# urgent-challenge/urgent2026_challenge_track1

Hardware: AMD Instinct MI355X
Metric: utterances/sec (4 s @ 48 kHz) train step (higher is better)
Workload: dtype bf16

## Files before the change

urgent2026_challenge_track1_amd/csrc/gemm.hip:

```cpp
#include <stdlib.h>

#include <type_traits>
#include "urse_common.h"

namespace urse {

typedef __bf16 bf16x8_t __attribute__((ext_vector_type(8)));
typedef short short8_t __attribute__((ext_vector_type(8)));
typedef short short4_t __attribute__((ext_vector_type(4)));
typedef float f32x4_t __attribute__((ext_vector_type(4)));

struct GemmDesc {
  const char* A;
  const char* B;
  char* C;
  const float* bias;
  const float* resid;
  long lda, ldb, ldc;
  long M, N, K;
  long ldr;
};

constexpr int BM = 128, BN = 128;
constexpr int SLAB = 64;
// ... 1409 lines not shown
        const long row = m0 + pass * RPP + lr_;
        const bool ok = slot < SLOTS && col < d.N && lr_ < RPP && row < d.M;
        gnb_xpre[i] = ok ? *reinterpret_cast<const float4*>(xt->gnb_x + row * d.ldc + col) : make_float4(0.f, 0.f, 0.f, 0.f);
      }
      if (slot < SLOTS && col < d.N) {
#pragma unroll
        for (int i = 0; i < XI; ++i) {
          const int lr_ = slot + i * SLOTS;
          const long row = m0 + pass * RPP + lr_;
          if (lr_ < RPP && row < d.M) {
            const float4 f = *reinterpret_cast<const float4*>(lds + lr_ * CP + chf * 16);
            __builtin_nontemporal_store(*reinterpret_cast<const f32x4_t*>(&f), reinterpret_cast<f32x4_t*>(C + row * d.ldc + col));
            const float4 xv = gnb_xpre[i];
            const bool first = row < gnb_bound;
            const float mean = first ? gnb_m[0] : gnb_m[1], rstd = first ? gnb_r[0] : gnb_r[1];
            const float dy[4] = {f.x, f.y, f.z, f.w}, xs[4] = {xv.x, xv.y, xv.z, xv.w};
            float a1 = 0.f, a2 = 0.f;
#pragma unroll
            for (int q = 0; q < 4; ++q) {
              const float xh = (xs[q] - mean) * rstd;
              gnb_dg[q] += dy[q] * xh;
              gnb_db[q] += dy[q];
              a1 += dy[q] * gnb_ga[q];
              a2 += dy[q] * gnb_ga[q] * xh;
            }
            if (first) { gsa += a1; gqa += a2; } else { gsb += a1; gqb += a2; }
          }
        }
      }
      continue;
    }
    int lrow = tid / CPR, ch = tid - lrow * CPR;
    constexpr int DROW = NTHR / CPR, DCH = NTHR - DROW * CPR;
    for (; lrow < RPP; lrow += DROW) {
      const long row = m0 + pass * RPP + lrow, col = n0 + ch * EPC;
      if (row < d.M && col < d.N) {
        const char* src = lds + lrow * CP + ch * 16;
        if (vec_ok && col + EPC <= d.N) {
          uint4 v = *reinterpret_cast<const uint4*>(src);
          if (OS == 4 && d.resid && ACT != 2) {
            const float4 rr = *reinterpret_cast<const float4*>(d.resid + row * d.ldr + col);
            float4 f = *reinterpret_cast<float4*>(&v);
            f.x += rr.x; f.y += rr.y; f.z += rr.z; f.w += rr.w;
            v = *reinterpret_cast<uint4*>(&f);
          }
          if (gst) {
            const float4 f = *reinterpret_cast<const float4*>(&v);
            const float sv = (f.x + f.y) + (f.z + f.w), qv = (f.x * f.x + f.y * f.y) + (f.z * f.z + f.w * f.w);
            if (row < gbound) { gsa += sv; gqa += qv; } else { gsb += sv; gqb += qv; }
          }
#ifdef NABL_NO_GST
          if (v.x == 0x12345678u)
#endif
          __builtin_nontemporal_store(*reinterpret_cast<const f32x4_t*>(&v), reinterpret_cast<f32x4_t*>(C + row * d.ldc + col));
          if constexpr (C2K) {
            if (C2) {
              float a0, a1, a2, a3, a4, a5, a6, a7;
              unpack2<f16_t>(v.x, a0, a1); unpack2<f16_t>(v.y, a2, a3); unpack2<f16_t>(v.z, a4, a5); unpack2<f16_t>(v.w, a6, a7);
              const uint4 o = make_uint4(pack2<bf16_t>(a0, a1), pack2<bf16_t>(a2, a3), pack2<bf16_t>(a4, a5), pack2<bf16_t>(a6, a7));
              __builtin_nontemporal_store(*reinterpret_cast<const f32x4_t*>(&o), reinterpret_cast<f32x4_t*>(C2 + row * d.ldr + col));
            }
          }
        } else {
          const TO* sv = reinterpret_cast<const TO*>(src);
          for (int e = 0; e < EPC && col + e < d.N; ++e) {
            float f = to_f32<TO>(sv[e]);
            if (OS == 4 && d.resid && ACT != 2) f += d.resid[row * d.ldr + col + e];
            if (gst) {
              if (row < gbound) { gsa += f; gqa += f * f; } else { gsb += f; gqb += f * f; }
            }
            C[row * d.ldc + col + e] = from_f32<TO>(f);
            if constexpr (C2K) {
              if (C2) C2[row * d.ldr + col + e] = f32_to_bf16(f);
            }
          }
        }
      }
      ch += DCH;
      if (ch >= CPR) { ch -= CPR; ++lrow; }
    }
  }
  if constexpr (GNB) {
    __syncthreads();
    constexpr int SLOTS = NTHR / CPR;
    double* red = reinterpret_cast<double*>(lds);
    float4* pg = reinterpret_cast<float4*>(lds + 1024);
    float4* pb = pg + SLOTS * CPR;
    const double r0 = wave_sum_d((double)gsa), r1 = wave_sum_d((double)gqa), r2 = wave_sum_d((double)gsb), r3 = wave_sum_d((double)gqb);
    if (lane == 0) { red[w * 4] = r0; red[w * 4 + 1] = r1; red[w * 4 + 2] = r2; red[w * 4 + 3] = r3; }
    if (tid < SLOTS * CPR) {
      pg[tid] = make_float4(gnb_dg[0], gnb_dg[1], gnb_dg[2], gnb_dg[3]);
      pb[tid] = make_float4(gnb_db[0], gnb_db[1], gnb_db[2], gnb_db[3]);
    }
    __syncthreads();
    if (tid < 4) {
      double t = 0.0;
      for (int i = 0; i < NWV; ++i) t += red[i * 4 + tid];
      const long g = gnb_g0 + (tid >> 1);
      if ((tid < 2 || gnb_bound < m0 + BMX) && g * xt->rpg < d.M) atomicAdd(xt->gnb_sums + g * 2 + (tid & 1), t);
    }
    if (tid >= 64 && tid < 64 + CPR) {
      const int chf = tid - 64;
      const long col = n0 + chf * EPC;
      if (col < d.N) {
        float4 sg = make_float4(0.f, 0.f, 0.f, 0.f), sb = sg;
        for (int i = 0; i < SLOTS; ++i) {
          const float4 a = pg[i * CPR + chf], bq = pb[i * CPR + chf];
          sg.x += a.x; sg.y += a.y; sg.z += a.z; sg.w += a.w;
          sb.x += bq.x; sb.y += bq.y; sb.z += bq.z; sb.w += bq.w;
        }
        float* part = xt->gnb_part + (long)(blockIdx.x % xt->gnb_slots) * 2 * d.N;
        const float vg[4] = {sg.x, sg.y, sg.z, sg.w}, vb[4] = {sb.x, sb.y, sb.z, sb.w};
        for (int q = 0; q < 4 && col + q < d.N; ++q) {
          atomicAdd(part + col + q, vg[q]);
          atomicAdd(part + d.N + col + q, vb[q]);
        }
      }
    }
    return;
  }
  if (gst) {
    __syncthreads();
    double* red = reinterpret_cast<double*>(lds);
    const double r0 = wave_sum_d((double)gsa), r1 = wave_sum_d((double)gqa), r2 = wave_sum_d((double)gsb), r3 = wave_sum_d((double)gqb);
    if (lane == 0) { red[w * 4] = r0; red[w * 4 + 1] = r1; red[w * 4 + 2] = r2; red[w * 4 + 3] = r3; }
    __syncthreads();
    if (tid < 4) {
      double t = 0.0;
      for (int i = 0; i < NWV; ++i) t += red[i * 4 + tid];
      const long g = gidx + (tid >> 1);
      if (tid < 2 || gbound < m0 + BMX) {
        if (g * rpg < d.M) atomicAdd(gstats + g * 2 + (tid & 1), t);
      }
    }
  }
}

template <typename TO, int NTW, int ACT, int BMX, int WNC = 2, typename TI = bf16_t>
__global__ void __launch_bounds__(BMX / 64 * WNC * 64) gemm_nt_dma_kernel(GemmDesc d, NtExtra x) {
  gemm_nt_dma_body<TO, NTW, ACT, BMX, WNC, 0, TI>(d, x.gstats, x.rpg);
}

__global__ void __launch_bounds__(512) gemm_nt_dma_gnb_kernel(GemmDesc d, NtExtra x) {
  gemm_nt_dma_body<float, 7, 0, 256, 2, 1>(d, nullptr, 0, &x);
}

__global__ void gnb_fold_kernel(const float* __restrict__ part, int slots, int N, float* __restrict__ dgamma, float* __restrict__ dbeta) {
  const int c = blockIdx.x * blockDim.x + threadIdx.x;
  if (c >= N) return;
  float a = 0.f, b = 0.f;
  for (int s = 0; s < slots; ++s) { a += part[(long)s * 2 * N + c]; b += part[(long)s * 2 * N + N + c]; }
  dgamma[c] += a;
  dbeta[c] += b;
}

template <typename TO, int ACT, typename TI = bf16_t>
__global__ void __launch_bounds__(512) gemm_nt_dma_grouped_kernel(const GemmDesc* __restrict__ descs) {
  const GemmDesc d = descs[blockIdx.y];
  gemm_nt_dma_body<TO, 7, ACT, 256, 2, 0, TI>(d);
}

template <int ACT, typename TI = bf16_t>
__global__ void __launch_bounds__(512) gemm_nt_bres_kernel(GemmDesc d, int wg_per_slice) {
  constexpr int BMX = 256, NTW = 7, BNX = 224, NST = 3, STAGE = BMX * 64, KSTEPS = 7, BRES = KSTEPS * 14 * 1024;
  __shared__ __attribute__((aligned(1024))) char lds[BRES + NST * STAGE];
  char* ring = lds + BRES;
  const int tm = (int)((d.M + BMX - 1) / BMX);
  const int tile_n = blockIdx.x / wg_per_slice, part = blockIdx.x - tile_n * wg_per_slice;
  const long n0 = (long)tile_n * BNX;
  const int tid = threadIdx.x, lane = tid & 63;
  const int w = __builtin_amdgcn_readfirstlane(tid >> 6), wm = w >> 1, wn = w & 1;
  const int nk = (int)(d.K / 32);
  const char* zsrc = reinterpret_cast<const char*>(g_tn_zero_page) + lane * 16;
  const int srow = lane >> 2, schunk = (lane & 3) ^ ((lane >> 3) & 3);
  const int lc = lane & 15, lr = lane >> 4;
  const int foff = lc * 64 + ((lr ^ ((lc >> 1) & 3)) << 4);
  for (int blk = w; blk < nk * 14; blk += 8) {
    const int kt = blk / 14, b = blk - kt * 14;
    const long row = n0 + b * 16 + srow;
    glds16(row < d.N ? d.B + (row * d.ldb) * 2 + schunk * 16 + (long)kt * 64 : zsrc, lds + blk * 1024);
  }
  f32x4_t bv[NTW];
#pragma unroll
  for (int j = 0; j < NTW; ++j) {
    const long col = n0 + (wn * NTW + j) * 16 + lr * 4;
#pragma unroll
    for (int r = 0; r < 4; ++r) bv[j][r] = (d.bias && col + r < d.N) ? d.bias[col + r] : 0.f;
  }
  bf16_t* C = reinterpret_cast<bf16_t*>(d.C);
  auto tile_src = [&](int mt, const char* (&pa)[2], bool (&aok)[2]) __attribute__((always_inline)) {
#pragma unroll
    for (int j = 0; j < 2; ++j) {
      const long row = (long)mt * BMX + 16 * (2 * w + j) + srow;
      aok[j] = mt < tm && row < d.M;
      pa[j] = d.A + (row * d.lda) * 2 + schunk * 16;
    }
  };
  auto issue = [&](const char* (&pa)[2], bool (&aok)[2], int kt, int slot) __attribute__((always_inline)) {
#pragma unroll
    for (int j = 0; j < 2; ++j)
      glds16((kt < nk && aok[j]) ? pa[j] + (long)kt * 64 : zsrc, ring + slot * STAGE + (2 * w + j) * 1024);
  };
  const char* pa[2];
  bool aok[2];
  tile_src(part, pa, aok);
  issue(pa, aok, 0, 2);
  for (int mt = part; mt < tm; mt += wg_per_slice) {
    const long m0 = (long)mt * BMX;
    issue(pa, aok, 1, 0);
    f32x4_t acc[4][NTW];
#pragma unroll
    for (int i = 0; i < 4; ++i)
#pragma unroll
      for (int j = 0; j < NTW; ++j) acc[i][j] = f32x4_t{0.f, 0.f, 0.f, 0.f};
    int slot = 2;
    for (int kt = 0; kt < nk; ++kt) {
      asm volatile("s_waitcnt vmcnt(2)" ::: "memory");
      __builtin_amdgcn_s_barrier();
      int nslot = slot + 2;
      if (nslot >= NST) nslot -= NST;
      issue(pa, aok, kt + 2, nslot);
      const char* As = ring + slot * STAGE + wm * 4096 + foff;
      const char* Bs = lds + kt * (14 * 1024) + wn * NTW * 1024 + foff;
      short8_t a[4], b[NTW];
#pragma unroll
      for (int i = 0; i < 4; ++i) a[i] = *reinterpret_cast<const short8_t*>(As + i * 1024);
#pragma unroll
      for (int j = 0; j < NTW; ++j) b[j] = *reinterpret_cast<const short8_t*>(Bs + j * 1024);
#pragma unroll
      for (int j = 0; j < NTW; ++j)
#pragma unroll
        for (int i = 0; i < 4; ++i) acc[i][j] = Frag<TI>::mma(b[j], a[i], acc[i][j]);
      if (++slot == NST) slot = 0;
    }
    asm volatile("s_waitcnt vmcnt(0)" ::: "memory");
    __syncthreads();
    tile_src(mt + wg_per_slice, pa, aok);
    issue(pa, aok, 0, 2);
    constexpr int CP = BNX * 2 + 16, RPP = 64, CPR = BNX / 8, DROW = 512 / CPR, DCH = 512 - DROW * CPR;
    static_assert(RPP * CP <= 2 * STAGE, "staging must leave slot 2 alone");
#pragma unroll 1
    for (int pass = 0; pass < BMX / RPP; ++pass) {
      if (pass > 0) {
        asm volatile("s_waitcnt lgkmcnt(0)" ::: "memory");
        __builtin_amdgcn_s_barrier();
      }
      if (wm == pass) {
#pragma unroll
        for (int j = 0; j < NTW; ++j) {
          const int lcol = (wn * NTW + j) * 16 + lr * 4;
#pragma unroll
          for (int i = 0; i < 4; ++i) {
            f32x4_t v = acc[i][j] + bv[j];
            if (ACT == 1) {
#pragma unroll
              for (int r = 0; r < 4; ++r) v[r] = tanhf_(v[r]);
            }
            uint2 pk;
            pk.x = pack2<TI>(v[0], v[1]);
            pk.y = pack2<TI>(v[2], v[3]);
            *reinterpret_cast<uint2*>(ring + (i * 16 + lc) * CP + lcol * 2) = pk;
          }
        }
      }
      asm volatile("s_waitcnt lgkmcnt(0)" ::: "memory");
      __builtin_amdgcn_s_barrier();
      int lrow = tid / CPR, ch = tid - lrow * CPR;
      for (; lrow < RPP; lrow += DROW) {
        const long row = m0 + pass * RPP + lrow, col = n0 + ch * 8;
        if (row < d.M && col < d.N) {
          const char* src = ring + lrow * CP + ch * 16;
          if (col + 8 <= d.N) {
            __builtin_nontemporal_store(*reinterpret_cast<const f32x4_t*>(src), reinterpret_cast<f32x4_t*>(C + row * d.ldc + col));
          } else {
            const bf16_t* sv = reinterpret_cast<const bf16_t*>(src);
            for (int e = 0; e < 8 && col + e < d.N; ++e) C[row * d.ldc + col + e] = sv[e];
          }
        }
        ch += DCH;
        if (ch >= CPR) { ch -= CPR; ++lrow; }
      }
    }
    asm volatile("s_waitcnt lgkmcnt(0)" ::: "memory");
    __builtin_amdgcn_s_barrier();
  }
  asm volatile("s_waitcnt vmcnt(0)" ::: "memory");
}

#ifdef URSE_EXPERIMENTS
constexpr int WR_ROWS = 32, WR_KS = 7, WR_NSLOT = 7, WR_STAGE = WR_KS * 2 * 1024, WR_BNX = 448, WR_CP = WR_BNX * 2 + 16, WR_AHEAD = WR_NSLOT - 1;
template <int ACT>
__global__ void __launch_bounds__(448) gemm_nt_wreg_kernel(GemmDesc d, int parts, long rows_per_part) {
  __shared__ __attribute__((aligned(1024))) char lds[WR_NSLOT * WR_STAGE + 2 * WR_ROWS * WR_CP];
  char* outs = lds + WR_NSLOT * WR_STAGE;
  const int tn_ = (int)gridDim.x / parts;
  const int lid = xcd_remap((int)blockIdx.x, (int)gridDim.x);
  const int part = lid / tn_, tile_n = lid - part * tn_;
  const long n0 = (long)tile_n * WR_BNX;
  const long r_begin = (long)part * rows_per_part;
  long r_end = r_begin + rows_per_part;
  if (r_end > d.M) r_end = d.M;
  if (r_begin >= r_end) return;
  const int nst = (int)((r_end - r_begin + WR_ROWS - 1) / WR_ROWS);
  const int tid = threadIdx.x, lane = tid & 63;
  const int w = __builtin_amdgcn_readfirstlane(tid >> 6);
  const int lc = lane & 15, lr = lane >> 4;
// ... 86 lines not shown
#endif
    }
    char* ob = outs + (k & 1) * (WR_ROWS * WR_CP);
#pragma unroll
    for (int i = 0; i < 2; ++i)
#pragma unroll
      for (int j = 0; j < 4; ++j) {
        f32x4_t v = acc[i][j] + bv[j];
        if (ACT == 1) {
#pragma unroll
          for (int r = 0; r < 4; ++r) v[r] = tanhf_(v[r]);
        }
        uint2 pk;
        pk.x = (unsigned)f32_to_bf16(v[0]) | ((unsigned)f32_to_bf16(v[1]) << 16);
        pk.y = (unsigned)f32_to_bf16(v[2]) | ((unsigned)f32_to_bf16(v[3]) << 16);
        *reinterpret_cast<uint2*>(ob + (i * 16 + lc) * WR_CP + (w * 64 + j * 16 + lr * 4) * 2) = pk;
      }
    {
      const int kk = k < 6 ? k : 6;
      switch (kk) {
        case 0: asm volatile("s_waitcnt vmcnt(10)" ::: "memory"); break;
        case 1: asm volatile("s_waitcnt vmcnt(14)" ::: "memory"); break;
        case 2: asm volatile("s_waitcnt vmcnt(18)" ::: "memory"); break;
        case 3: asm volatile("s_waitcnt vmcnt(22)" ::: "memory"); break;
        case 4: asm volatile("s_waitcnt vmcnt(26)" ::: "memory"); break;
        case 5: asm volatile("s_waitcnt vmcnt(30)" ::: "memory"); break;
        default: asm volatile("s_waitcnt vmcnt(34)" ::: "memory"); break;
      }
    }
    static_assert(WR_AHEAD == 6 && NPC == 4, "the counted waits above are written for six stages ahead and four stores per sweep");
    asm volatile("s_waitcnt lgkmcnt(0)" ::: "memory");
    __builtin_amdgcn_s_barrier();
  }
  sweep(nst - 1);
}
#endif

static int check_desc_host(const GemmDesc& d, int es, const char* who) {
  URSE_CHECK_ARG(d.A && d.B && d.C, "%s: null operand", who);
  URSE_CHECK_ARG(d.M > 0 && d.N > 0 && d.K > 0, "%s: empty problem", who);
  URSE_CHECK_ARG((d.K * es) % SLAB == 0, "%s: K (%ld) must be a multiple of %d elements", who, d.K, SLAB / es);
  URSE_CHECK_ARG((d.lda * es) % 16 == 0 && (d.ldb * es) % 16 == 0 && ((uintptr_t)d.A % 16) == 0 &&
                     ((uintptr_t)d.B % 16) == 0,
                 "%s: operands must be 16-byte aligned with 16-byte-multiple row pitch", who);
  URSE_CHECK_ARG(d.lda >= d.K && d.ldb >= d.K && d.ldc >= d.N, "%s: leading dimension too small", who);
  return URSE_OK;
}

template <typename T, typename TO>
static void launch_nt(const GemmDesc* descs, const GemmDesc& single, int groups, int max_blocks, int act,
                      hipStream_t st) {
  hipLaunchKernelGGL((gemm_nt_kernel<T, TO>), dim3(max_blocks, 1, groups), dim3(256), 0, st, descs, single, act);
}

static int dispatch_nt(const GemmDesc* descs, const GemmDesc& single, int groups, int max_blocks, int in_dtype,
                       int out_dtype, int act, hipStream_t st) {
  if (in_dtype == URSE_BF16 && out_dtype == URSE_BF16) launch_nt<bf16_t, bf16_t>(descs, single, groups, max_blocks, act, st);
  else if (in_dtype == URSE_BF16 && out_dtype == URSE_F32) launch_nt<bf16_t, float>(descs, single, groups, max_blocks, act, st);
  else if (in_dtype == URSE_F32 && out_dtype == URSE_F32) launch_nt<float, float>(descs, single, groups, max_blocks, act, st);
  else if (in_dtype == URSE_F32 && out_dtype == URSE_BF16) launch_nt<float, bf16_t>(descs, single, groups, max_blocks, act, st);
  else if (in_dtype == URSE_F16 && out_dtype == URSE_F16) launch_nt<f16_t, f16_t>(descs, single, groups, max_blocks, act, st);
  else if (in_dtype == URSE_F16 && out_dtype == URSE_F32) launch_nt<f16_t, float>(descs, single, groups, max_blocks, act, st);
  else { set_error("gemm_nt: bad dtype %d/%d", in_dtype, out_dtype); return URSE_ERR_INVALID_ARG; }
  URSE_CHECK_LAUNCH("urse_gemm_nt");
  return URSE_OK;
}

static long g_nt_bres_min_n = getenv("URSE_NT_BRES_MIN_N") ? atol(getenv("URSE_NT_BRES_MIN_N")) : 448;
static int g_nt_bres_wgs = 256;
static int g_nt_wide_default = 1;
static long g_nt_wide_maxk = 256;

static int gemm_nt_impl(const void* A, int64_t lda, const void* B, int64_t ldb, void* C, int64_t ldc,
                        const float* bias, const float* resid, int64_t ldr, int64_t M, int64_t N, int64_t K,
                        int in_dtype, int out_dtype, int act, void* stream, double* gstats, long rpg, int* fused) {
  NtExtra xtra{};
  GemmDesc d;
  d.A = (const char*)A; d.B = (const char*)B; d.C = (char*)C; d.bias = bias; d.resid = resid;
  d.lda = lda; d.ldb = ldb; d.ldc = ldc; d.M = M; d.N = N; d.K = K; d.ldr = ldr;
  const bool in16 = in_dtype == URSE_BF16 || in_dtype == URSE_F16;
  const bool f16 = in_dtype == URSE_F16;
  URSE_CHECK_ARG(in16 || in_dtype == URSE_F32, "urse_gemm_nt: bad operand dtype %d", in_dtype);
  URSE_CHECK_ARG(out_dtype == URSE_F32 || (out_dtype == URSE_BF16 && !f16) || (out_dtype == URSE_F16 && f16),
                 "urse_gemm_nt: output dtype %d with operand dtype %d (16-bit outputs take the operands' format)", out_dtype, in_dtype);
  const bool out16 = out_dtype != URSE_F32;
  int rc = check_desc_host(d, in16 ? 2 : 4, "urse_gemm_nt");
  if (rc) return rc;
  URSE_CHECK_ARG(!resid || act == 2 || out_dtype == URSE_F32 || (in_dtype == URSE_F16 && out_dtype == URSE_F16 && act == 1),
                 "urse_gemm_nt: residual epilogue writes f32 (f16 operands with act 1: the aux slot is the bf16 copy of the output)");
  URSE_CHECK_ARG(act != 2 || resid, "urse_gemm_nt: act 2 (tanh backward) needs the aux operand");
  static const bool no_dma = getenv("URSE_NT_NO_DMA") != nullptr;
  const char* bres_env = getenv("URSE_NT_BRES");
  const int bres_mode = bres_env ? atoi(bres_env) : 1;
#ifdef URSE_EXPERIMENTS
  const long wreg_min_n = getenv("URSE_NT_WREG_MIN_N") ? atol(getenv("URSE_NT_WREG_MIN_N")) : 0;
  if (wreg_min_n > 0 && in_dtype == URSE_BF16 && out_dtype == URSE_BF16 && !no_dma && M >= 8192 && N >= wreg_min_n && K == 32 * WR_KS &&
      !resid && act != 2 && (ldc * 2) % 16 == 0 && ((uintptr_t)C % 16) == 0 && M * lda * 2 < 0xFFFFF000L && M * ldc * 2 < 0xFFFFF000L) {
    const int tn = (int)((N + WR_BNX - 1) / WR_BNX);
    int parts = 252 / tn;
    if (parts < 1) parts = 1;
    long rpp = (M + parts - 1) / parts;
    rpp = (rpp + WR_ROWS - 1) / WR_ROWS * WR_ROWS;
    dim3 grid((unsigned)(tn * parts));
    hipStream_t st = (hipStream_t)stream;
    note_launch(URSE_KV_NT_BRES);
    if (act == 0) hipLaunchKernelGGL(gemm_nt_wreg_kernel<0>, grid, dim3(448), 0, st, d, parts, rpp);
    else hipLaunchKernelGGL(gemm_nt_wreg_kernel<1>, grid, dim3(448), 0, st, d, parts, rpp);
    URSE_CHECK_LAUNCH("urse_gemm_nt");
    return URSE_OK;
  }
#endif
  if (bres_mode && in16 && out16 && !no_dma && M >= 8192 && N >= g_nt_bres_min_n && K % 32 == 0 &&
      K >= 96 && K <= 224 && !resid && act != 2 && (ldc * 2) % 16 == 0 && ((uintptr_t)C % 16) == 0) {
    const int tn = (int)((N + 223) / 224);
    int per = g_nt_bres_wgs / tn;
    if (per < 1) per = 1;
    dim3 grid((unsigned)(tn * per));
    hipStream_t st = (hipStream_t)stream;
    note_launch(URSE_KV_NT_BRES);
    if (f16) {
      if (act == 0) hipLaunchKernelGGL((gemm_nt_bres_kernel<0, f16_t>), grid, dim3(512), 0, st, d, per);
      else hipLaunchKernelGGL((gemm_nt_bres_kernel<1, f16_t>), grid, dim3(512), 0, st, d, per);
    } else if (act == 0) hipLaunchKernelGGL(gemm_nt_bres_kernel<0>, grid, dim3(512), 0, st, d, per);
    else hipLaunchKernelGGL(gemm_nt_bres_kernel<1>, grid, dim3(512), 0, st, d, per);
    URSE_CHECK_LAUNCH("urse_gemm_nt");
    return URSE_OK;
  }
  if (in16 && !no_dma && M >= 2048 && N >= 160 && K % 32 == 0 && K >= 96 && !(f16 && act == 2)) {
    const long pad7 = (N + 223) / 224 * 224, pad8 = (N + 255) / 256 * 256;
    int ntw = pad7 <= pad8 ? 7 : 8;
    if (const char* e = getenv("URSE_NT_NTW")) ntw = atoi(e) == 8 ? 8 : 7;
    int bmx = 256;
    if (const char* e = getenv("URSE_NT_BMX")) bmx = atoi(e) == 128 ? 128 : 256;
    int wide = g_nt_wide_default && K <= g_nt_wide_maxk && N >= 1792 && out_dtype == URSE_BF16 && (N + 447) / 448 * 448 <= pad7 + 64;
    if (const char* e = getenv("URSE_NT_WIDE")) wide = atoi(e) != 0 && N >= 448;
    if (f16) { wide = 0; bmx = 256; }
    const long tl = wide ? ((M + 127) / 128) * ((N + 447) / 448) : ((M + bmx - 1) / bmx) * ((N + 32L * ntw - 1) / (32L * ntw));
    URSE_CHECK_ARG(tl < (1L << 31), "urse_gemm_nt: too many tiles");
    dim3 grid((unsigned)tl);
    hipStream_t st = (hipStream_t)stream;
    if (gstats && out_dtype == URSE_F32 && act != 2 && !wide && rpg >= bmx) {
      xtra.gstats = gstats;
      xtra.rpg = rpg;
      if (fused) *fused = 1;
    }
#define URSE_NT_DMA(TO_, NTW_, ACT_, BMX_) \
  hipLaunchKernelGGL((gemm_nt_dma_kernel<TO_, NTW_, ACT_, BMX_>), grid, dim3(BMX_ * 2), 0, st, d, xtra)
#define URSE_NT_DMA_W(TO_, ACT_) \
  hipLaunchKernelGGL((gemm_nt_dma_kernel<TO_, 7, ACT_, 128, 4>), grid, dim3(512), 0, st, d, xtra)
#define URSE_NT_DMA_B(TO_, NTW_, ACT_) do { if (wide) URSE_NT_DMA_W(TO_, ACT_); else if (bmx == 128) URSE_NT_DMA(TO_, NTW_, ACT_, 128); else URSE_NT_DMA(TO_, NTW_, ACT_, 256); } while (0)
#define URSE_NT_DMA_ACT(TO_, NTW_) \
  do { if (act == 0) URSE_NT_DMA_B(TO_, NTW_, 0); else if (act == 1) URSE_NT_DMA_B(TO_, NTW_, 1); else URSE_NT_DMA_B(TO_, NTW_, 2); } while (0)
    note_launch(wide ? URSE_KV_NT_RING_WIDE : URSE_KV_NT_RING);
    if (f16) {
#define URSE_NT_DMA_H(TO_, NTW_, ACT_) hipLaunchKernelGGL((gemm_nt_dma_kernel<TO_, NTW_, ACT_, 256, 2, f16_t>), grid, dim3(512), 0, st, d, xtra)
#define URSE_NT_DMA_H_ACT(TO_, NTW_) do { if (act == 0) URSE_NT_DMA_H(TO_, NTW_, 0); else URSE_NT_DMA_H(TO_, NTW_, 1); } while (0)
      if (out_dtype == URSE_F16) { if (ntw == 7) URSE_NT_DMA_H_ACT(f16_t, 7); else URSE_NT_DMA_H_ACT(f16_t, 8); }
      else { if (ntw == 7) URSE_NT_DMA_H_ACT(float, 7); else URSE_NT_DMA_H_ACT(float, 8); }
    } else if (out_dtype == URSE_BF16) {
      if (ntw == 7) URSE_NT_DMA_ACT(bf16_t, 7); else URSE_NT_DMA_ACT(bf16_t, 8);
    } else {
      if (ntw == 7) URSE_NT_DMA_ACT(float, 7); else URSE_NT_DMA_ACT(float, 8);
    }
    URSE_CHECK_LAUNCH("urse_gemm_nt");
    return URSE_OK;
  }
  const long blocks = ((M + BM - 1) / BM) * ((N + BN - 1) / BN);
  URSE_CHECK_ARG(blocks < (1L << 31), "urse_gemm_nt: too many tiles");
  note_launch(URSE_KV_NT_128);
  return dispatch_nt(nullptr, d, 1, (int)blocks, in_dtype, out_dtype, act, (hipStream_t)stream);
}

extern "C" int urse_gemm_nt(const void* A, int64_t lda, const void* B, int64_t ldb, void* C, int64_t ldc,
                            const float* bias, const float* resid, int64_t ldr, int64_t M, int64_t N, int64_t K,
                            int in_dtype, int out_dtype, int act, void* stream) {
  return gemm_nt_impl(A, lda, B, ldb, C, ldc, bias, resid, ldr, M, N, K, in_dtype, out_dtype, act, stream, nullptr, 0, nullptr);
}

extern "C" int urse_gemm_nt_gnstats(const void* A, int64_t lda, const void* B, int64_t ldb, float* C, int64_t ldc,
                                    const float* bias, const float* resid, int64_t ldr, int64_t M, int64_t N, int64_t K,
                                    int in_dtype, int act, double* stats, int64_t rows_per_group, void* stream) {
  URSE_CHECK_ARG(stats && rows_per_group > 0 && M % rows_per_group == 0 && ldc == N && N % 4 == 0,
                 "urse_gemm_nt_gnstats: needs whole groups of rows, a dense output and N %% 4 == 0");
  const int groups = (int)(M / rows_per_group);
  (void)hipMemsetAsync(stats, 0, sizeof(double) * 2 * groups, (hipStream_t)stream);
  int fused = 0;
  int rc = gemm_nt_impl(A, lda, B, ldb, C, ldc, bias, resid, ldr, M, N, K, in_dtype, URSE_F32, act, stream, stats, rows_per_group,
                        &fused);
  if (rc || fused) return rc;
  return urse_groupnorm_stats(C, stats, groups, (int)rows_per_group, 1, (int)N, (int)N, stream);
}

extern "C" int urse_gemm_nt_gnbwd(const void* A, int64_t lda, const void* B, int64_t ldb, float* C, int64_t M, int64_t N, int64_t K,
                                  int in_dtype, const float* x, const double* stats, const float* gamma, double* sums, float* dgamma,
                                  float* dbeta, float* part, int slots, int64_t rows_per_group, float eps, void* stream) {
  URSE_CHECK_ARG(A && B && C && x && stats && gamma && sums && dgamma && dbeta && part && slots > 0 && rows_per_group > 0,
                 "urse_gemm_nt_gnbwd: bad argument");
  static const bool no_dma = getenv("URSE_NT_NO_DMA") != nullptr;
  if (no_dma || in_dtype != URSE_BF16 || M < 2048 || N < 160 || N > 224 || N % 4 || K % 32 || K < 96 || rows_per_group < 256 ||
      M % rows_per_group || ((uintptr_t)C % 16) || ((uintptr_t)x % 16)) {
    set_error("urse_gemm_nt_gnbwd: shape M%ld N%ld K%ld not served by the fused kernel", (long)M, (long)N, (long)K);
    return URSE_ERR_UNSUPPORTED;
  }
  GemmDesc d;
  d.A = (const char*)A; d.B = (const char*)B; d.C = (char*)C; d.bias = nullptr; d.resid = nullptr;
  d.lda = lda; d.ldb = ldb; d.ldc = N; d.M = M; d.N = N; d.K = K; d.ldr = 0;
  int rc = check_desc_host(d, 2, "urse_gemm_nt_gnbwd");
  if (rc) return rc;
  hipStream_t st = (hipStream_t)stream;
  const size_t sums_bytes = sizeof(double) * 2 * (size_t)(M / rows_per_group), part_bytes = sizeof(float) * 2 * (size_t)N * slots;
  if (reinterpret_cast<char*>(part) == reinterpret_cast<char*>(sums) + sums_bytes) {
    (void)hipMemsetAsync(sums, 0, sums_bytes + part_bytes, st);
  } else {
    (void)hipMemsetAsync(sums, 0, sums_bytes, st);
    (void)hipMemsetAsync(part, 0, part_bytes, st);
  }
  NtExtra xt{};
  xt.rpg = rows_per_group; xt.gnb_x = x; xt.gnb_stats = stats; xt.gnb_gamma = gamma; xt.gnb_sums = sums; xt.gnb_part = part;
  xt.gnb_slots = slots; xt.gnb_eps = eps;
  const long tl = (M + 255) / 256;
  URSE_CHECK_ARG(tl < (1L << 31), "urse_gemm_nt_gnbwd: too many tiles");
  note_launch(URSE_KV_NT_RING);
  hipLaunchKernelGGL(gemm_nt_dma_gnb_kernel, dim3((unsigned)tl), dim3(512), 0, st, d, xt);
  hipLaunchKernelGGL(gnb_fold_kernel, dim3((unsigned)((N + 255) / 256)), dim3(256), 0, st, part, slots, (int)N, dgamma, dbeta);
  URSE_CHECK_LAUNCH("urse_gemm_nt_gnbwd");
  return URSE_OK;
}

extern "C" int urse_gemm_nt_grouped(const void* descs, int groups, int max_blocks, int in_dtype, int out_dtype,
                                    int act, void* stream) {
  URSE_CHECK_ARG(descs && groups > 0 && max_blocks > 0, "urse_gemm_nt_grouped: bad argument");
  GemmDesc dummy;
  memset(&dummy, 0, sizeof(dummy));
  note_launch(URSE_KV_NT_GROUPED_128);
  return dispatch_nt((const GemmDesc*)descs, dummy, groups, max_blocks, in_dtype, out_dtype, act,
                     (hipStream_t)stream);
}

extern "C" int urse_gemm_nt_grouped_h(const void* descs, const int64_t* host_descs, int groups, int in_dtype,
                                      int out_dtype, int act, void* stream) {
  URSE_CHECK_ARG(descs && host_descs && groups > 0 && groups < 65536, "urse_gemm_nt_grouped_h: bad argument");
  const GemmDesc* hd = reinterpret_cast<const GemmDesc*>(host_descs);
  const bool f16 = in_dtype == URSE_F16;
  const int es = (in_dtype == URSE_BF16 || f16) ? 2 : 4;
  URSE_CHECK_ARG(out_dtype == URSE_F32 || (out_dtype == URSE_BF16 && !f16) || (out_dtype == URSE_F16 && f16),
                 "urse_gemm_nt_grouped_h: output dtype %d with operand dtype %d", out_dtype, in_dtype);
  bool dma = es == 2 && !(f16 && act == 2) && !getenv("URSE_NT_NO_DMA") && !getenv("URSE_NT_GROUPED_NO_DMA");
  long t128 = 0, tdma = 0;
  const char* mm = getenv("URSE_NT_GROUPED_MIN_M");
  const long min_m = mm ? atol(mm) : 1024;
  for (int g = 0; g < groups; ++g) {
    const GemmDesc& d = hd[g];
    if (int rc = check_desc_host(d, es, "urse_gemm_nt_grouped_h")) return rc;
    dma = dma && d.K % 32 == 0 && d.N >= 160 && d.M >= min_m;
    t128 = std::max(t128, ((d.M + BM - 1) / BM) * ((d.N + BN - 1) / BN));
    tdma = std::max(tdma, ((d.M + 255) / 256) * ((d.N + 223) / 224));
  }
  URSE_CHECK_ARG(t128 < (1L << 31), "urse_gemm_nt_grouped_h: too many tiles");
  if (!dma) {
    GemmDesc dummy;
    memset(&dummy, 0, sizeof(dummy));
    note_launch(URSE_KV_NT_GROUPED_128);
    return dispatch_nt((const GemmDesc*)descs, dummy, groups, (int)t128, in_dtype, out_dtype, act, (hipStream_t)stream);
  }
  dim3 grid((unsigned)tdma, (unsigned)groups);
  hipStream_t st = (hipStream_t)stream;
  const GemmDesc* dd = (const GemmDesc*)descs;
#define URSE_NT_G(TO_, ACT_) hipLaunchKernelGGL((gemm_nt_dma_grouped_kernel<TO_, ACT_>), grid, dim3(512), 0, st, dd)
#define URSE_NT_G_ACT(TO_) do { if (act == 0) URSE_NT_G(TO_, 0); else if (act == 1) URSE_NT_G(TO_, 1); else URSE_NT_G(TO_, 2); } while (0)
  note_launch(URSE_KV_NT_GROUPED_RING);
#define URSE_NT_GH(TO_, ACT_) hipLaunchKernelGGL((gemm_nt_dma_grouped_kernel<TO_, ACT_, f16_t>), grid, dim3(512), 0, st, dd)
  if (f16 && out_dtype == URSE_F16) { if (act == 0) URSE_NT_GH(f16_t, 0); else URSE_NT_GH(f16_t, 1); }
  else if (f16) { if (act == 0) URSE_NT_GH(float, 0); else URSE_NT_GH(float, 1); }
  else if (out_dtype == URSE_BF16) URSE_NT_G_ACT(bf16_t);
  else if (out_dtype == URSE_F32) URSE_NT_G_ACT(float);
  else { set_error("urse_gemm_nt_grouped_h: bad output dtype %d", out_dtype); return URSE_ERR_INVALID_ARG; }
  URSE_CHECK_LAUNCH("urse_gemm_nt_grouped_h");
  return URSE_OK;
}


extern "C" int urse_gemm_tn(const void* A, int64_t lda, const void* B, int64_t ldb, float* C, int64_t ldc,
                            float* colsum, int64_t R, int64_t Mo, int64_t No, int64_t shift, int64_t inner,
                            int64_t period, int64_t invalid_step, int64_t perm_h, int dtype, int target_workgroups,
                            void* stream) {
  URSE_CHECK_ARG(A && B && C && R > 0 && Mo > 0 && No > 0 && target_workgroups >= 0, "urse_gemm_tn: bad argument");
  const long g_tn_target_wgs = target_workgroups > 0 ? target_workgroups : 256;
  const bool act_f16 = dtype == URSE_BF16_ACT_F16;
  if (act_f16) {
    if (!urse_gemm_tn_act_f16_supported(R, Mo, No, 0, colsum != nullptr, 1, 0) || perm_h != 0 || shift != 0 || period != 0) {
      set_error("urse_gemm_tn: URSE_BF16_ACT_F16 serves the shapes urse_gemm_tn_act_f16_supported accepts (R%ld Mo%ld No%ld)", (long)R, (long)Mo, (long)No);
      return URSE_ERR_UNSUPPORTED;
    }
    dtype = URSE_BF16;
  }
  const int es = dtype == URSE_BF16 ? 2 : 4;
  URSE_CHECK_ARG((lda * es) % 16 == 0 && (ldb * es) % 16 == 0 && ((uintptr_t)A % 16) == 0 && ((uintptr_t)B % 16) == 0,
                 "urse_gemm_tn: operands must be 16-byte aligned with 16-byte-multiple row pitch");
  URSE_CHECK_ARG(lda >= Mo && ldb >= No && ldc >= No, "urse_gemm_tn: leading dimension too small");
  TnArgs p;
  p.A = (const char*)A; p.B = (const char*)B; p.C = C; p.colsum = colsum;
  p.lda = lda; p.ldb = ldb; p.ldc = ldc; p.R = R; p.Mo = Mo; p.No = No;
  p.shift = shift; p.inner = inner > 0 ? inner : 1; p.period = period; p.invalid_step = invalid_step;
  p.perm_h = perm_h;
  p.B2 = nullptr; p.C2 = nullptr; p.ldb2 = p.ldc2 = p.No2 = p.nt1 = 0; p.pad_[0] = p.pad_[1] = 0;
  static const bool no_dma = getenv("URSE_TN_NO_DMA") != nullptr;
  if (dtype == URSE_BF16 && !no_dma && perm_h == 0 && shift == 0 && period == 0 && Mo < 512 && Mo >= 160 && No >= 512 &&
      R >= 16384 && R < (1L << 30)) {
    TnArgs q = p;
    q.A = (const char*)B; q.lda = ldb; q.Mo = No;
    q.B = (const char*)A; q.ldb = lda; q.No = Mo;
    q.perm_h = TN_TRANSPOSED;
    const long pad7 = (q.No + 223) / 224 * 224, pad8 = (q.No + 255) / 256 * 256;
    const int ntw = pad7 < pad8 ? 7 : 8;
    const long bnx = 32L * ntw;
    const long tl = ((q.Mo + 255) / 256) * ((q.No + bnx - 1) / bnx);
    long slices = g_tn_target_wgs / tl;
    if (slices < 1) slices = 1;
    long rps = (R + slices - 1) / slices;
    rps = (rps + 31) / 32 * 32;
    slices = (R + rps - 1) / rps;
    q.rows_per_slice = rps;
    dim3 grid((unsigned)(tl * slices));
    note_launch(URSE_KV_TN_RING_T);
    if (act_f16) note_launch(URSE_KV_TN_ACT_F16);
    launch_tn_dma(ntw, colsum ? 2 : 0, grid, (hipStream_t)stream, q, act_f16 ? 1 : 0);
    URSE_CHECK_LAUNCH("urse_gemm_tn");
    return URSE_OK;
  }
  if (dtype == URSE_BF16 && !no_dma && Mo >= 512 && No >= 160 && R >= 16384 && inner < (1L << 31) && R < (1L << 30) && shift > -(1L << 30) && shift < (1L << 30) && period < (1L << 31)) {
    const long pad7 = (No + 223) / 224 * 224, pad8 = (No + 255) / 256 * 256;
    const int ntw = pad7 < pad8 ? 7 : 8;
    const long bnx = 32L * ntw;
    const long tl = ((Mo + 255) / 256) * ((No + bnx - 1) / bnx);
    long slices = g_tn_target_wgs / tl;
    if (slices < 1) slices = 1;
    long rps = (R + slices - 1) / slices;
    rps = (rps + 31) / 32 * 32;
    slices = (R + rps - 1) / rps;
    p.rows_per_slice = rps;
    dim3 grid((unsigned)(tl * slices));
    note_launch(URSE_KV_TN_RING);
    launch_tn_dma(ntw, colsum ? 1 : 0, grid, (hipStream_t)stream, p);
    URSE_CHECK_LAUNCH("urse_gemm_tn");
    return URSE_OK;
  }
  const long tiles = ((Mo + BM - 1) / BM) * ((No + BN - 1) / BN);
  const int bkr = dtype == URSE_BF16 ? 32 : 16;
  long target = 768;
  if (const char* e = getenv("URSE_TN_TARGET")) target = atol(e);
  long slices = target / tiles;
  const long max_slices = (R + 4 * bkr - 1) / (4 * bkr);
  if (slices > max_slices) slices = max_slices;
  if (slices < 1) slices = 1;
  long rps = (R + slices - 1) / slices;
  rps = (rps + bkr - 1) / bkr * bkr;
  slices = (R + rps - 1) / rps;
  p.rows_per_slice = rps;
  URSE_CHECK_ARG(tiles * slices < (1L << 31), "urse_gemm_tn: too many tiles");
  dim3 grid((unsigned)(tiles * slices));
  note_launch(URSE_KV_TN_128);
  if (dtype == URSE_BF16) hipLaunchKernelGGL(gemm_tn_kernel<bf16_t>, grid, dim3(256), 0, (hipStream_t)stream, p);
  else hipLaunchKernelGGL(gemm_tn_kernel<float>, grid, dim3(256), 0, (hipStream_t)stream, p);
  URSE_CHECK_LAUNCH("urse_gemm_tn");
  return URSE_OK;
}

extern "C" int urse_gemm_tn_grouped(const void* descs, int groups, int max_blocks, int dtype, void* stream) {
  URSE_CHECK_ARG(descs && groups > 0 && max_blocks > 0 && groups < 65536, "urse_gemm_tn_grouped: bad argument");
  dim3 grid((unsigned)max_blocks, (unsigned)groups);
  note_launch(URSE_KV_TN_GROUPED);
  if (dtype == URSE_BF16)
    hipLaunchKernelGGL(gemm_tn_grouped_kernel<bf16_t>, grid, dim3(256), 0, (hipStream_t)stream, (const TnArgs*)descs);
  else
    hipLaunchKernelGGL(gemm_tn_grouped_kernel<float>, grid, dim3(256), 0, (hipStream_t)stream, (const TnArgs*)descs);
  URSE_CHECK_LAUNCH("urse_gemm_tn_grouped");
// ... 103 lines not shown
```

Before: 249.5.

## Add persistent NT GEMM kernel that prefetches next tile during epilogue

Adds a persistent-workgroup variant of the 256x224 NT GEMM (bf16/f16 in, f32 out) that loops over tiles with a stride of the grid size. It issues the next tile's first two K-stages into spare LDS slots while the current tile's epilogue (bias, residual, group-stat accumulation) runs, which hides launch and pipeline-fill cost. It also reuses bias registers across tiles that share a column. The plain path uses it by default when the shape and alignment conditions hold and there are more tiles than 256 workgroups. The GroupNorm-backward fused variant stays opt-in through an environment variable. The risks are load imbalance from a fixed 256-workgroup grid and heavier register and LDS pressure.

```diff
diff --git a/urgent2026_challenge_track1_amd/csrc/gemm.hip b/urgent2026_challenge_track1_amd/csrc/gemm.hip
--- a/urgent2026_challenge_track1_amd/csrc/gemm.hip
+++ b/urgent2026_challenge_track1_amd/csrc/gemm.hip
@@ -1585,6 +1585,312 @@
   for (int s = 0; s < slots; ++s) { a += part[(long)s * 2 * N + c]; b += part[(long)s * 2 * N + N + c]; }
   dgamma[c] += a;
   dbeta[c] += b;
+}
+
+__device__ __forceinline__ void lds_barrier() {
+  asm volatile("s_waitcnt lgkmcnt(0)" ::: "memory");
+  __builtin_amdgcn_s_barrier();
+  asm volatile("" ::: "memory");
+}
+
+template <int GNB, typename TI>
+__device__ __forceinline__ void gemm_nt_dma_pers_body(const GemmDesc& d, const NtExtra& xt) {
+  constexpr int NTW = 7, BMX = 256, BNX = 224, NWV = 8, NTHR = 512, NST = 4, STAGE = (BMX + 256) * 64, BOFF = BMX * 64;
+  constexpr int CP = BNX * 4 + 16, RPP = 64, NPASS = BMX / RPP, CPR = BNX / 4;
+  static_assert(RPP * CP <= 2 * STAGE, "the staging must leave slots 2-3 to the next tile's first stages");
+  __shared__ __attribute__((aligned(1024))) char lds[NST * STAGE];
+  const int tn = (int)((d.N + BNX - 1) / BNX), tm = (int)((d.M + BMX - 1) / BMX), tiles = tm * tn;
+  const int tid = threadIdx.x, lane = tid & 63;
+  const int w = __builtin_amdgcn_readfirstlane(tid >> 6), wm = w >> 1, wn = w & 1;
+  const int nk = (int)(d.K / 32);
+  const char* zsrc = reinterpret_cast<const char*>(g_tn_zero_page) + lane * 16;
+  const int srow = lane >> 2, schunk = (lane & 3) ^ ((lane >> 3) & 3);
+  const int lc = lane & 15, lr = lane >> 4;
+  const int foff = lc * 64 + ((lr ^ ((lc >> 1) & 3)) << 4);
+  float* C = reinterpret_cast<float*>(d.C);
+
+  const char* pa[2];
+  const char* pb[2];
+  bool aok[2], bok[2];
+  long m0n = 0, n0n = 0;
+  auto tile_src = [&](int v) __attribute__((always_inline)) {
+    const bool live = v < tiles;
+    const int bid = live ? xcd_remap(v, tiles) : 0;
+    const int tile_m = bid / tn, tile_n = bid - tile_m * tn;
+    m0n = (long)tile_m * BMX;
+    n0n = (long)tile_n * BNX;
+#pragma unroll
+    for (int j = 0; j < 2; ++j) {
+      const int rowl = 16 * (2 * w + j) + srow;
+      aok[j] = live && m0n + rowl < d.M;
+      pa[j] = d.A + ((m0n + rowl) * d.lda) * 2 + schunk * 16;
+      bok[j] = live && rowl < BNX && n0n + rowl < d.N;
+      pb[j] = d.B + ((n0n + rowl) * d.ldb) * 2 + schunk * 16;
+    }
+  };
+  auto issue = [&](int kt, int slot) __attribute__((always_inline)) {
+    char* sbase = lds + slot * STAGE;
+#pragma unroll
+    for (int j = 0; j < 2; ++j) glds16(aok[j] ? pa[j] + (long)kt * 64 : zsrc, sbase + (2 * w + j) * 1024);
+#pragma unroll
+    for (int j = 0; j < 2; ++j) glds16(bok[j] ? pb[j] + (long)kt * 64 : zsrc, sbase + BOFF + (2 * w + j) * 1024);
+  };
+
+  int v = blockIdx.x;
+  if (v >= tiles) return;
+  tile_src(v);
+  issue(0, 2);
+  issue(1, 3);
+
+  f32x4_t bv[NTW];
+  float gnb_ga[4] = {0.f, 0.f, 0.f, 0.f};
+  long n0b = -1;
+  const bool gst = !GNB && xt.gstats != nullptr;
+  constexpr int SLOTS = NTHR / CPR, DCH = NTHR - SLOTS * CPR, RI = RPP * CPR / NTHR, XI = (RPP + SLOTS - 1) / SLOTS;
+  static_assert(RI * NTHR == RPP * CPR, "a pass is a whole number of sweep iterations");
+
+  for (; v < tiles; v += gridDim.x) {
+    const long m0 = m0n, n0 = n0n;
+    issue(2, 0);
+    f32x4_t acc[4][NTW];
+#pragma unroll
+    for (int i = 0; i < 4; ++i)
+#pragma unroll
+      for (int j = 0; j < NTW; ++j) acc[i][j] = f32x4_t{0.f, 0.f, 0.f, 0.f};
+
+    int slot = 2;
+    for (int kt = 0; kt < nk; ++kt) {
+      if (kt + 2 < nk) asm volatile("s_waitcnt vmcnt(8)" ::: "memory");
+      else if (kt + 1 < nk) asm volatile("s_waitcnt vmcnt(4)" ::: "memory");
+      else asm volatile("s_waitcnt vmcnt(0)" ::: "memory");
+      __builtin_amdgcn_s_barrier();
+      if (kt + 3 < nk) issue(kt + 3, (slot + 3) & 3);
+      const char* As = lds + slot * STAGE + wm * 4096 + foff;
+      const char* Bs = lds + slot * STAGE + BOFF + wn * NTW * 1024 + foff;
+      short8_t a[4], b[NTW];
+#pragma unroll
+      for (int i = 0; i < 4; ++i) a[i] = *reinterpret_cast<const short8_t*>(As + i * 1024);
+#pragma unroll
+      for (int j = 0; j < NTW; ++j) b[j] = *reinterpret_cast<const short8_t*>(Bs + j * 1024);
+#pragma unroll
+      for (int j = 0; j < NTW; ++j)
+#pragma unroll
+        for (int i = 0; i < 4; ++i) acc[i][j] = Frag<TI>::mma(b[j], a[i], acc[i][j]);
+      slot = (slot + 1) & 3;
+    }
+    const long gnb_g0 = GNB ? m0 / xt.rpg : 0, gnb_bound = GNB ? (gnb_g0 + 1) * xt.rpg : 0;
+    double gnb_st[4] = {0.0, 0.0, 0.0, 0.0};
+    float gnb_m[2] = {0.f, 0.f}, gnb_r[2] = {0.f, 0.f};
+    if constexpr (GNB) {
+      const long glast = d.M / xt.rpg - 1;
+#pragma unroll
+      for (int q = 0; q < 2; ++q) {
+        const long g = gnb_g0 + q < glast ? gnb_g0 + q : glast;
+        gnb_st[2 * q] = xt.gnb_stats[g * 2];
+        gnb_st[2 * q + 1] = xt.gnb_stats[g * 2 + 1];
+      }
+    }
+    lds_barrier();
+    if constexpr (GNB) {
+      const double cnt = (double)xt.rpg * (double)d.N;
+#pragma unroll
+      for (int q = 0; q < 2; ++q) {
+        const double mu = gnb_st[2 * q] / cnt;
+        double var = gnb_st[2 * q + 1] / cnt - mu * mu;
+        if (var < 0.0) var = 0.0;
+        gnb_m[q] = (float)mu;
+        gnb_r[q] = (float)(1.0 / sqrt(var + (double)xt.gnb_eps));
+        asm volatile("" : "+v"(gnb_m[q]), "+v"(gnb_r[q]));
+      }
+    }
+    if (n0 != n0b) {
+      n0b = n0;
+      if constexpr (GNB) {
+        const long col = n0 + (tid % CPR) * 4;
+#pragma unroll
+        for (int q = 0; q < 4; ++q) {
+          gnb_ga[q] = (col + q < d.N) ? xt.gnb_gamma[col + q] : 0.f;
+          asm volatile("" : "+v"(gnb_ga[q]));
+        }
+      } else {
+#pragma unroll
+        for (int j = 0; j < NTW; ++j) {
+          const long col = n0 + (wn * NTW + j) * 16 + lr * 4;
+#pragma unroll
+          for (int r = 0; r < 4; ++r) bv[j][r] = (d.bias && col + r < d.N) ? d.bias[col + r] : 0.f;
+          asm volatile("" : "+v"(bv[j]));
+        }
+      }
+    }
+    tile_src(v + (int)gridDim.x);
+    issue(0, 2);
+    issue(1, 3);
+
+    float gsa = 0.f, gqa = 0.f, gsb = 0.f, gqb = 0.f;
+    float gnb_dg[4] = {0.f, 0.f, 0.f, 0.f}, gnb_db[4] = {0.f, 0.f, 0.f, 0.f};
+    const long gidx = gst ? m0 / xt.rpg : 0, gbound = gst ? (gidx + 1) * xt.rpg : 0;
+#pragma unroll 1
+    for (int pass = 0; pass < NPASS; ++pass) {
+      if (pass > 0) lds_barrier();
+      float4 pre[GNB ? XI : RI];
+      auto arrived = [](float4& q) __attribute__((always_inline)) { asm volatile("" : "+v"(q.x), "+v"(q.y), "+v"(q.z), "+v"(q.w)); };
+      int t = tid;
+      asm volatile("" : "+v"(t));
+      const int slot0 = t / CPR, ch0 = t - slot0 * CPR;
+      const long prow = m0 + pass * RPP;
+      const int rows = d.M - prow < RPP ? (int)(d.M - prow) : RPP;
+      const int chunks = d.N - n0 < BNX ? (int)((d.N - n0) / 4) : CPR;
+      const unsigned ldc32 = (unsigned)d.ldc, ldr32 = (unsigned)d.ldr;
+      float* cbase = C + prow * d.ldc + n0;
+      const int xrow0 = (slot0 + SLOTS - (pass & 1) * (RPP % SLOTS)) % SLOTS;
+      if constexpr (GNB) {
+        const float* xbase = xt.gnb_x + prow * d.ldc + n0;
+#pragma unroll
+        for (int i = 0; i < XI; ++i) {
+          const int lr_ = xrow0 + i * SLOTS;
+          const bool ok = slot0 < SLOTS && ch0 < chunks && lr_ < rows;
+          pre[i] = *reinterpret_cast<const float4*>(ok ? reinterpret_cast<const char*>(xbase + ((unsigned)lr_ * ldc32 + (unsigned)ch0 * 4u)) : zsrc);
+        }
+      } else {
+        const float* rbase = d.resid ? d.resid + prow * d.ldr + n0 : nullptr;
+        int lrow = slot0, ch = ch0;
+#pragma unroll
+        for (int i = 0; i < RI; ++i) {
+          const bool ok = rbase && lrow < rows && ch < chunks;
+          pre[i] = *reinterpret_cast<const float4*>(ok ? reinterpret_cast<const char*>(rbase + ((unsigned)lrow * ldr32 + (unsigned)ch * 4u)) : zsrc);
+          lrow += SLOTS;
+          ch += DCH;
+          if (ch >= CPR) { ch -= CPR; ++lrow; }
+        }
+      }
+      if (wm == pass) {
+#pragma unroll
+        for (int j = 0; j < NTW; ++j) {
+          const int lcol = (wn * NTW + j) * 16 + lr * 4;
+#pragma unroll
+          for (int i = 0; i < 4; ++i)
+            *reinterpret_cast<f32x4_t*>(lds + (i * 16 + lc) * CP + lcol * 4) = acc[i][j] + (GNB ? f32x4_t{0.f, 0.f, 0.f, 0.f} : bv[j]);
+        }
+      }
+      lds_barrier();
+#pragma unroll
+      for (int i = 0; i < (GNB ? XI : RI); ++i) arrived(pre[i]);
+      if constexpr (GNB) {
+        {
+#pragma unroll
+          for (int i = 0; i < XI; ++i) {
+            const int lr_ = xrow0 + i * SLOTS;
+            if (slot0 < SLOTS && ch0 < chunks && lr_ < rows) {
+              const float4 f = *reinterpret_cast<const float4*>(lds + lr_ * CP + ch0 * 16);
+              __builtin_nontemporal_store(*reinterpret_cast<const f32x4_t*>(&f),
+                                          reinterpret_cast<f32x4_t*>(cbase + ((unsigned)lr_ * ldc32 + (unsigned)ch0 * 4u)));
+              const float4 xv = pre[i];
+              const bool first = prow + lr_ < gnb_bound;
+              const float mean = first ? gnb_m[0] : gnb_m[1], rstd = first ? gnb_r[0] : gnb_r[1];
+              const float dy[4] = {f.x, f.y, f.z, f.w}, xs[4] = {xv.x, xv.y, xv.z, xv.w};
+              float a1 = 0.f, a2 = 0.f;
+#pragma unroll
+              for (int q = 0; q < 4; ++q) {
+                const float xh = (xs[q] - mean) * rstd;
+                gnb_dg[q] += dy[q] * xh;
+                gnb_db[q] += dy[q];
+                a1 += dy[q] * gnb_ga[q];
+                a2 += dy[q] * gnb_ga[q] * xh;
+              }
+              if (first) { gsa += a1; gqa += a2; } else { gsb += a1; gqb += a2; }
+            }
+          }
+        }
+      } else {
+        int lrow = slot0, ch = ch0;
+#pragma unroll
+        for (int i = 0; i < RI; ++i) {
+          if (lrow < rows && ch < chunks) {
+            float4 f = *reinterpret_cast<const float4*>(lds + lrow * CP + ch * 16);
+            if (d.resid) {
+              const float4 rr = pre[i];
+              f.x += rr.x; f.y += rr.y; f.z += rr.z; f.w += rr.w;
+            }
+            if (gst) {
+              const float sv = (f.x + f.y) + (f.z + f.w), qv = (f.x * f.x + f.y * f.y) + (f.z * f.z + f.w * f.w);
+              if (prow + lrow < gbound) { gsa += sv; gqa += qv; } else { gsb += sv; gqb += qv; }
+            }
+            __builtin_nontemporal_store(*reinterpret_cast<const f32x4_t*>(&f),
+                                        reinterpret_cast<f32x4_t*>(cbase + ((unsigned)lrow * ldc32 + (unsigned)ch * 4u)));
+          }
+          lrow += SLOTS;
+          ch += DCH;
+          if (ch >= CPR) { ch -= CPR; ++lrow; }
+        }
+      }
+    }
+    lds_barrier();
+    if (GNB || gst) {
+      double* red = reinterpret_cast<double*>(lds);
+      float4* pg = reinterpret_cast<float4*>(lds + 1024);
+      float4* pbb = pg + SLOTS * CPR;
+      const double r0 = wave_sum_d((double)gsa), r1 = wave_sum_d((double)gqa), r2 = wave_sum_d((double)gsb), r3 = wave_sum_d((double)gqb);
+      if (lane == 0) { red[w * 4] = r0; red[w * 4 + 1] = r1; red[w * 4 + 2] = r2; red[w * 4 + 3] = r3; }
+      if constexpr (GNB) {
+        if (tid < SLOTS * CPR) {
+          pg[tid] = make_float4(gnb_dg[0], gnb_dg[1], gnb_dg[2], gnb_dg[3]);
+          pbb[tid] = make_float4(gnb_db[0], gnb_db[1], gnb_db[2], gnb_db[3]);
+        }
+      }
+      lds_barrier();
+      if (tid < 4) {
+        double t = 0.0;
+        for (int i = 0; i < NWV; ++i) t += red[i * 4 + tid];
+        if constexpr (GNB) {
+          const long g = gnb_g0 + (tid >> 1);
+          if ((tid < 2 || gnb_bound < m0 + BMX) && g * xt.rpg < d.M) atomicAdd(xt.gnb_sums + g * 2 + (tid & 1), t);
+        } else {
+          const long g = gidx + (tid >> 1);
+          if ((tid < 2 || gbound < m0 + BMX) && g * xt.rpg < d.M) atomicAdd(xt.gstats + g * 2 + (tid & 1), t);
+        }
+      }
+      if constexpr (GNB) {
+        if (tid >= 64 && tid < 64 + CPR) {
+          const int chf = tid - 64;
+          const long col = n0 + chf * 4;
+          if (col < d.N) {
+            float4 sg = make_float4(0.f, 0.f, 0.f, 0.f), sb = sg;
+            for (int i = 0; i < SLOTS; ++i) {
+              const float4 a = pg[i * CPR + chf], bq = pbb[i * CPR + chf];
+              sg.x += a.x; sg.y += a.y; sg.z += a.z; sg.w += a.w;
+              sb.x += bq.x; sb.y += bq.y; sb.z += bq.z; sb.w += bq.w;
+            }
+            float* part = xt.gnb_part + (long)(v % xt.gnb_slots) * 2 * d.N;
+            const float vg[4] = {sg.x, sg.y, sg.z, sg.w}, vb[4] = {sb.x, sb.y, sb.z, sb.w};
+            for (int q = 0; q < 4 && col + q < d.N; ++q) {
+              atomicAdd(part + col + q, vg[q]);
+              atomicAdd(part + d.N + col + q, vb[q]);
+            }
+          }
+        }
+      }
+      lds_barrier();
+    }
+  }
+  asm volatile("s_waitcnt vmcnt(0)" ::: "memory");
+}
+
+template <typename TI>
+__global__ void __launch_bounds__(512) gemm_nt_dma_pers_kernel(GemmDesc d, NtExtra x) {
+  gemm_nt_dma_pers_body<0, TI>(d, x);
+}
+
+__global__ void __launch_bounds__(512) gemm_nt_dma_gnb_pers_kernel(GemmDesc d, NtExtra x) {
+  gemm_nt_dma_pers_body<1, bf16_t>(d, x);
+}
+
+static int nt_persist_wgs(long tiles, bool dflt) {
+  const char* e = getenv("URSE_NT_PERSIST");
+  if (e ? atoi(e) == 0 : !dflt) return 0;
+  const char* g = getenv("URSE_NT_PERSIST_WGS");
+  long wgs = g ? atol(g) : 256;
+  if (wgs < 1) wgs = 1;
+  return tiles > wgs ? (int)wgs : 0;
 }
 
 template <typename TO, int ACT, typename TI = bf16_t>
@@ -1977,6 +2283,14 @@
 #define URSE_NT_DMA_ACT(TO_, NTW_) \
   do { if (act == 0) URSE_NT_DMA_B(TO_, NTW_, 0); else if (act == 1) URSE_NT_DMA_B(TO_, NTW_, 1); else URSE_NT_DMA_B(TO_, NTW_, 2); } while (0)
     note_launch(wide ? URSE_KV_NT_RING_WIDE : URSE_KV_NT_RING);
+    const int pers = (!wide && bmx == 256 && ntw == 7 && out_dtype == URSE_F32 && act == 0 && N % 4 == 0 && ldc % 4 == 0 && ((uintptr_t)C % 16) == 0 &&
+                      ldc < (1L << 24) && (!resid || (ldr % 4 == 0 && ldr < (1L << 24) && ((uintptr_t)resid % 16) == 0))) ? nt_persist_wgs(tl, true) : 0;
+    if (pers) {
+      if (f16) hipLaunchKernelGGL(gemm_nt_dma_pers_kernel<f16_t>, dim3((unsigned)pers), dim3(512), 0, st, d, xtra);
+      else hipLaunchKernelGGL(gemm_nt_dma_pers_kernel<bf16_t>, dim3((unsigned)pers), dim3(512), 0, st, d, xtra);
+      URSE_CHECK_LAUNCH("urse_gemm_nt");
+      return URSE_OK;
+    }
     if (f16) {
 #define URSE_NT_DMA_H(TO_, NTW_, ACT_) hipLaunchKernelGGL((gemm_nt_dma_kernel<TO_, NTW_, ACT_, 256, 2, f16_t>), grid, dim3(512), 0, st, d, xtra)
 #define URSE_NT_DMA_H_ACT(TO_, NTW_) do { if (act == 0) URSE_NT_DMA_H(TO_, NTW_, 0); else URSE_NT_DMA_H(TO_, NTW_, 1); } while (0)
@@ -2046,7 +2360,8 @@
   const long tl = (M + 255) / 256;
   URSE_CHECK_ARG(tl < (1L << 31), "urse_gemm_nt_gnbwd: too many tiles");
   note_launch(URSE_KV_NT_RING);
-  hipLaunchKernelGGL(gemm_nt_dma_gnb_kernel, dim3((unsigned)tl), dim3(512), 0, st, d, xt);
+  if (const int pers = nt_persist_wgs(tl, false)) hipLaunchKernelGGL(gemm_nt_dma_gnb_pers_kernel, dim3((unsigned)pers), dim3(512), 0, st, d, xt);
+  else hipLaunchKernelGGL(gemm_nt_dma_gnb_kernel, dim3((unsigned)tl), dim3(512), 0, st, d, xt);
   hipLaunchKernelGGL(gnb_fold_kernel, dim3((unsigned)((N + 255) / 256)), dim3(256), 0, st, part, slots, (int)N, dgamma, dbeta);
   URSE_CHECK_LAUNCH("urse_gemm_nt_gnbwd");
   return URSE_OK;
```

Measured after the change: 251.7 (median of 6 runs). No clear change (+0.9%).
